# ZhonghuaYi/EI-Nexus_official

Hardware: AMD Instinct MI355X
Metric: event-image pairs/s (extract+match, 346x260, 1024 kpts) (higher is better)
Workload: dtype f32; 1 GPU; B32 346x260 5-bin event voxel + gray image, VGG(event)+SuperPoint(image) extractors, MNN matcher, k=1024; global_batch=32, event_bins=5, parallelism=dp1 (pairs sharded, metric all-reduce only), log_assignment=False, dense_outputs=False, same_scene_pairs=False, weights=seeded synthetic, descriptor-head bias calibrated (per-channel mean removed)

## Files before the change

### ei-nexus_official_amd/_lib.py

```python
import ctypes
import os

_HERE = os.path.dirname(os.path.abspath(__file__))
LIB_PATH = os.environ.get("EINX_LIB") or os.path.join(_HERE, "libeinx_hip.so")

c_void_p, c_int, c_float, c_size_t, c_char_p = ctypes.c_void_p, ctypes.c_int, ctypes.c_float, ctypes.c_size_t, ctypes.c_char_p


class ConvDesc(ctypes.Structure):
    _fields_ = [("w_native", c_void_p), ("bias", c_void_p), ("scale", c_void_p), ("shift", c_void_p),
                ("cin", ctypes.c_int32), ("cout", ctypes.c_int32), ("ks", ctypes.c_int32), ("relu", ctypes.c_int32),
                ("pool", ctypes.c_int32)]


class DetectParams(ctypes.Structure):
    _fields_ = [("B", ctypes.c_int32), ("Hp", ctypes.c_int32), ("Wp", ctypes.c_int32), ("H", ctypes.c_int32),
                ("W", ctypes.c_int32), ("h0", ctypes.c_int32), ("w0", ctypes.c_int32), ("radius", ctypes.c_int32),
                ("top_k", ctypes.c_int32), ("det_thr", c_float), ("ordering_xy", ctypes.c_int32), ("cap", ctypes.c_int32),
                ("nms_iters", ctypes.c_int32)]


class ExtractorDesc(ctypes.Structure):
    _fields_ = [("struct_size", c_size_t), ("cell", ctypes.c_int32), ("n_backbone", ctypes.c_int32), ("n_det", ctypes.c_int32), ("n_desc", ctypes.c_int32),
                ("backbone", ctypes.POINTER(ConvDesc)), ("det_head", ctypes.POINTER(ConvDesc)), ("desc_head", ctypes.POINTER(ConvDesc)),
# ... 34 lines not shown
class GtMatchesParams(ctypes.Structure):
    _fields_ = [("struct_size", c_size_t)] + [(n, ctypes.c_int32) for n in ("B", "cap0", "cap1", "cols0", "cols1", "kp_yx", "H0", "W0", "H1", "W1",
                                                                            "homography")] + [("pos_sq", c_float), ("neg_sq", c_float)]


class EventArrays(ctypes.Structure):
    _fields_ = [("x", c_void_p), ("y", c_void_p), ("t", c_void_p), ("p", c_void_p), ("x_type", ctypes.c_int32), ("y_type", ctypes.c_int32),
                ("t_type", ctypes.c_int32), ("p_type", ctypes.c_int32), ("n", ctypes.c_int64)]


class LgLayer(ctypes.Structure):
    _names = ("Wqkv", "bqkv", "Wo", "bo", "sf0_w", "sf0_b", "sln_g", "sln_b", "sf3_w", "sf3_b",
              "Wqk", "bqk", "Wv", "bv", "Wco", "bco", "cf0_w", "cf0_b", "cln_g", "cln_b", "cf3_w", "cf3_b", "Wqk_v", "bqk_v")
    _fields_ = [(n, c_void_p) for n in _names]


class LgWeights(ctypes.Structure):
    _fields_ = [("struct_size", c_size_t), ("layer_size", c_size_t), ("in_w", c_void_p), ("in_b", c_void_p), ("Wr", c_void_p), ("proj_w", c_void_p), ("proj_b", c_void_p),
                ("match_w", c_void_p), ("match_b", c_void_p), ("n_layers", ctypes.c_int32), ("heads", ctypes.c_int32),
                ("d", ctypes.c_int32), ("input_dim", ctypes.c_int32), ("filter_threshold", c_float),
                ("layers", ctypes.POINTER(LgLayer))]


class LgHead(ctypes.Structure):
    _fields_ = [(n, c_void_p) for n in ("proj_w", "proj_b", "match_w", "match_b", "token_w", "token_b")]


SIGNATURES = {
    "einx_version": (c_char_p, []),
    "einx_abi_version": (c_int, []),
    "einx_build_flags": (c_char_p, []),
    "einx_params_hash": (c_int, [c_void_p, c_int, c_void_p, c_void_p, c_void_p, c_void_p]),
    "einx_last_error": (c_char_p, []),
    "einx_math_eval": (c_int, [c_int, c_void_p, ctypes.c_longlong, c_void_p, c_void_p]),
    "einx_fork_stream_of": (c_void_p, [c_void_p]),
    "einx_fork_stream_prepare_beside": (c_int, [c_void_p, ctypes.POINTER(c_void_p), c_int]),
    "einx_stream_overlap_us": (c_int, [c_void_p, c_void_p, c_int, ctypes.POINTER(ctypes.c_float)]),
    "einx_device_count": (c_int, []),
    "einx_profile_enable": (c_int, [c_int]),
    "einx_profile_report": (c_int, [c_char_p, c_size_t]),
    "einx_extractor_create": (c_void_p, [ctypes.POINTER(ExtractorDesc)]),
    "einx_extractor_destroy": (None, [c_void_p]),
    "einx_fork_stream_prepare": (c_int, [c_void_p]),
    "einx_fork_stream_release": (c_int, [c_void_p]),
    "einx_fork_stream_count": (c_int, []),
    "einx_side_stream": (c_void_p, [c_void_p, c_int, ctypes.POINTER(c_void_p), c_int]),
    "einx_extract_shapes": (c_int, [c_void_p, c_int, c_int, ctypes.POINTER(ExtractShapes)]),
    "einx_extract_ws_bytes": (c_size_t, [c_void_p, c_int, c_int, c_int, c_int, c_int]),
    "einx_extract": (c_int, [c_void_p, c_void_p, c_void_p, c_int, c_int, c_int, c_int, c_void_p, c_size_t, ctypes.POINTER(ExtractOut), c_void_p]),
    "einx_extract_watch": (c_int, [c_void_p, c_void_p, c_void_p, c_int, c_int, c_int, c_int, c_void_p, c_size_t, ctypes.POINTER(ExtractOut),
                           ctypes.POINTER(WeightWatch), c_void_p]),
    "einx_conv_last_kernel": (c_char_p, []),
    "einx_conv_plan": (c_char_p, [c_int] * 11),
    "einx_conv_weight_elems": (c_size_t, [c_int, c_int, c_int]),
    "einx_conv_repack": (c_int, [c_void_p, c_int, c_int, c_int, c_void_p, c_void_p]),
    "einx_bn_fold": (c_int, [c_void_p, c_void_p, c_void_p, c_void_p, c_float, c_int, c_void_p, c_void_p, c_void_p]),
    "einx_conv_block": (c_int, [c_void_p, c_int, c_int, c_int, c_int, c_int, c_int, c_int, ctypes.POINTER(ConvDesc), c_void_p, c_void_p]),
    "einx_conv_first_two_fused_ok": (c_int, [ctypes.POINTER(ConvDesc), ctypes.POINTER(ConvDesc), c_int, c_int, c_int]),
    "einx_conv_first_two_fused": (c_int, [c_void_p, c_int, c_int, c_int, c_int, c_int, c_int, c_int, ctypes.POINTER(ConvDesc), ctypes.POINTER(ConvDesc),
                                  c_void_p, c_void_p]),
    "einx_div_inplace": (c_int, [c_void_p, c_size_t, c_float, c_void_p]),
    "einx_image_prepare": (c_int, [c_void_p, c_int, c_int, c_int, c_int, ctypes.c_longlong, ctypes.c_longlong, ctypes.c_longlong, ctypes.c_longlong,
                           c_float, c_void_p, c_void_p]),
    "einx_score_map": (c_int, [c_void_p, c_int, c_int, c_int, c_int, c_void_p, c_int, c_int, c_int, c_int, c_int, c_int, c_void_p,
                               c_void_p, c_void_p]),
    "einx_remove_border": (c_int, [c_void_p, c_int, c_int, c_int, c_int, c_void_p]),
    "einx_detect_ws_bytes": (c_size_t, [ctypes.POINTER(DetectParams)]),
    "einx_detect": (c_int, [c_void_p, ctypes.POINTER(DetectParams), c_void_p, c_void_p, c_void_p, c_void_p, c_void_p, c_void_p,
                            c_void_p, c_void_p]),
    "einx_desc_sample": (c_int, [c_void_p, c_int, c_int, c_int, c_int, c_int, c_int, c_int, c_int, c_void_p, c_void_p, c_int, c_float,
                                 c_void_p, c_void_p]),
    "einx_normalize_map": (c_int, [c_void_p, c_int, c_int, c_int, c_float, c_void_p, c_void_p, c_void_p]),
    "einx_upsample_ws_bytes": (c_size_t, [c_int, c_int, c_int]),
    "einx_upsample_normalize": (c_int, [c_void_p, c_int, c_int, c_int, c_int, c_int, c_int, c_int, c_int, c_int, c_int, c_float,
                                        c_void_p, c_void_p, c_size_t, c_void_p]),
    "einx_mnn_ws_bytes": (c_size_t, [c_int, c_int, c_int]),
    "einx_mnn": (c_int, [c_void_p, c_void_p, c_int, c_void_p, c_void_p, c_int, c_int, c_int, c_void_p, c_void_p, c_void_p, c_void_p,
                         c_void_p, c_void_p, c_void_p]),
    "einx_mnn_gather": (c_int, [c_void_p, c_void_p, c_int, c_void_p, c_void_p, c_int, c_int, c_int, c_void_p, c_void_p, c_void_p, c_void_p,
                                c_void_p, c_void_p, c_void_p, c_void_p, c_int, c_void_p, c_void_p, c_void_p, c_void_p]),
    "einx_mnn_thresh": (c_int, [c_void_p, c_void_p, c_int, c_void_p, c_void_p, c_int, c_int, c_int, c_int, c_float, c_int, c_float, c_void_p,
                                c_void_p, c_void_p, c_void_p, c_void_p, c_void_p, c_void_p]),
    "einx_gather_matches": (c_int, [c_void_p, c_void_p, c_void_p, c_void_p, c_int, c_int, c_int, c_int, c_void_p, c_void_p, c_void_p,
                                    c_void_p]),
    "einx_events_ws_bytes": (c_size_t, [c_int, c_int, c_int]),
    "einx_voxel_ws_bytes": (c_size_t, [c_int, c_int, c_int, c_int, ctypes.c_int64]),
    "einx_voxel_grid": (c_int, [c_void_p, c_void_p, c_void_p, c_void_p, c_void_p, c_int, c_int, c_int, c_int, c_int, c_void_p, c_void_p,
                                c_size_t, c_void_p]),
    "einx_events_mask": (c_int, [c_void_p, c_void_p, c_void_p, c_int, c_int, c_int, c_void_p, c_void_p, c_void_p]),
    "einx_time_surface_ws_bytes": (c_size_t, [c_int, c_int, c_int, c_int, ctypes.c_int64]),
    "einx_event_stack_ws_bytes": (c_size_t, [c_int, c_int, c_int, c_int, ctypes.c_int64]),
    "einx_distance_map_ws_bytes": (c_size_t, [c_int, c_int, c_int, c_int, ctypes.c_int64]),
    "einx_time_surface": (c_int, [c_void_p, c_void_p, c_void_p, c_void_p, c_void_p, c_int, c_int, c_int, c_int, c_void_p, c_void_p, c_size_t,
                                  c_void_p]),
    "einx_event_stack": (c_int, [c_void_p, c_void_p, c_void_p, c_void_p, c_void_p, c_int, c_int, c_int, c_int, c_void_p, c_void_p, c_size_t,
                                 c_void_p]),
    "einx_distance_map": (c_int, [c_void_p, c_void_p, c_void_p, c_void_p, c_void_p, c_int, c_int, c_int, c_int, c_void_p, c_void_p, c_size_t,
                                  c_void_p]),
    "einx_distance_map_plan": (c_char_p, [c_int, c_int]),
    "einx_events_windows_ws_bytes": (c_size_t, [c_int, c_int, c_int]),
    "einx_voxel_windows_ws_bytes": (c_size_t, [c_int, c_int, c_int, c_int, ctypes.c_int64]),
    "einx_voxel_grid_windows": (c_int, [c_void_p, c_void_p, c_void_p, c_void_p, ctypes.c_int64, c_void_p, c_void_p, c_int, c_int, c_int, c_int, c_int,
                                        c_void_p, c_void_p, c_size_t, c_void_p]),
    "einx_events_mask_windows": (c_int, [c_void_p, c_void_p, ctypes.c_int64, c_void_p, c_void_p, c_int, c_int, c_int, c_void_p, c_size_t, c_void_p,
                                         c_void_p]),
    "einx_events_pack": (c_int, [ctypes.POINTER(EventArrays), c_int, c_void_p, c_void_p, c_void_p, c_void_p, c_void_p, c_int]),
# ... 74 lines not shown
```

### ei-nexus_official_amd/csrc/conv.hip

```cpp
#include <stdio.h>
#include <stdlib.h>

#include <type_traits>

#include "einx_common.h"

namespace {

constexpr int kCoutTile = 64;

struct ConvArgs {
  const float* in;
  const float* w;
  const float* bias;
  const float* scale;
  const float* shift;
  float* out;
  int B, Cin, Cout, CoutPad;
  int Hs, Ws, h0, w0;
  int H, W;
  int tilesX, tilesY;
  int relu;
};

constexpr bool pitch_conflict_free(int th, int tw, int pitch) {
  const int npix = th * tw;
  for (int q0 = 0; q0 < npix; q0 += 32) {
    unsigned used = 0;
    for (int q = q0; q < q0 + 32 && q < npix; ++q) {
      const unsigned bit = 1u << (((q / tw) * pitch + q % tw) & 31);
      if (used & bit) return false;
      used |= bit;
    }
  }
  return true;
}
constexpr int conv_lds_pitch(int th, int tw) {
  for (int p = tw + 2; p < tw + 2 + 32; ++p)
    if (pitch_conflict_free(th, tw, p)) return p;
  return tw + 2;
}

template <int X>
__device__ __forceinline__ float lane_xor(float v) {
  const int i = __builtin_bit_cast(int, v);
  if constexpr (X == 1) return __builtin_bit_cast(float, __builtin_amdgcn_update_dpp(0, i, 0xB1, 0xF, 0xF, true));
  else if constexpr (X == 8) return __builtin_bit_cast(float, __builtin_amdgcn_update_dpp(0, i, 0x128, 0xF, 0xF, true));
  else if constexpr (X == 16) return __builtin_bit_cast(float, __builtin_amdgcn_ds_swizzle(i, 0x401F));
  else return __shfl_xor(v, X, 64);
}

template <int X>
__device__ __forceinline__ float max_lane_xor(float v) {
  if constexpr (X == 1) {
    float r;
    asm("s_nop 1\n\tv_max_f32_dpp %0, %1, %1 quad_perm:[1,0,3,2] row_mask:0xf bank_mask:0xf bound_ctrl:1" : "=v"(r) : "v"(v));
    return r;
  } else if constexpr (X == 8) {
    float r;
    asm("s_nop 1\n\tv_max_f32_dpp %0, %1, %1 row_ror:8 row_mask:0xf bank_mask:0xf bound_ctrl:1" : "=v"(r) : "v"(v));
    return r;
  } else {
    return fmaxf(v, lane_xor<X>(v));
  }
}

__device__ __forceinline__ __amdgpu_buffer_rsrc_t conv_rsrc(const void* p, unsigned bytes) {
  return __builtin_amdgcn_make_buffer_rsrc(const_cast<void*>(p), 0, (int)bytes, 0x00020000);
}

constexpr int conv_stage_groups(int nthr, int plane_e, int ck) {
  int ng = nthr / plane_e;
  while (ng > 1 && ck % ng != 0) --ng;
  return ng < 1 ? 1 : ng;
}

template <int KS, int TH, int TW, int WM, int WN, int MT, int NT, int CK, bool POOL, bool XTRA = false, int WPS = (CK < 8 ? 6 : 1)>
__global__ __launch_bounds__(WM * WN * 64, WPS) void conv_block_kernel(const ConvArgs a) {
  constexpr int kMT = MT, kNT = NT;
  constexpr int NW = WM * WN;
  constexpr int TAPS = KS * KS;
  constexpr int HALO = KS / 2;
  constexpr int PW = TW + 2 * HALO;
  constexpr int PH = TH + 2 * HALO;
  constexpr int PITCH = KS == 1 ? PW : conv_lds_pitch(TH, TW);
  constexpr int PLANE = PH * PITCH;
  constexpr int PLANE_E = PH * PW;
  constexpr int NTHR = NW * 64;
  constexpr int NPIX = TH * TW;
  static_assert(WM * MT * 32 == kCoutTile, "a workgroup covers 64 output channels");
  static_assert(WN * NT * 32 >= NPIX, "tile does not fit the workgroup's pixel slots");
  static_assert(KS == 1 || NPIX >= 32, "unused slots alias the slot one run earlier");
  static_assert(CK % 2 == 0, "channels are consumed in pairs");
  static_assert(PLANE_E <= NTHR, "one staging thread per halo position");
  constexpr int NG = conv_stage_groups(NTHR, PLANE_E, CK);
  constexpr int CPT = CK / NG;
  constexpr int IN_LDS = CK * PLANE;
  static_assert(IN_LDS % 4 == 0, "the weight tile behind the input tile is float4 aligned");
  constexpr int W_ROWS = CK * TAPS;
  constexpr int W_F4 = W_ROWS * kCoutTile / 4;
  constexpr int W_PER_THR = (W_F4 + NTHR - 1) / NTHR;
  constexpr int LDS_FLOATS = IN_LDS + W_ROWS * kCoutTile;

  __shared__ __attribute__((aligned(16))) float lds[LDS_FLOATS];
  __shared__ __attribute__((aligned(16))) float s_bias[kCoutTile], s_scale[kCoutTile], s_shift[kCoutTile];
  float* in_tile = lds;
  float* w_tile = lds + IN_LDS;

  const int tid = threadIdx.x;
  const int wave = __builtin_amdgcn_readfirstlane(tid >> 6);
  const int wm = wave / WN, wn = wave % WN;
  const int lane = tid & 63;
  const int half = lane >> 5;
  const int j = lane & 31;

  const int ncot = (int)gridDim.y;
  int item = xcd_contiguous((int)(blockIdx.x + blockIdx.y * gridDim.x), (int)gridDim.x * ncot);
  const int co0 = (item % ncot) * kCoutTile;
  int bid = item / ncot;
  const int tx_i = bid % a.tilesX;
  bid /= a.tilesX;
  const int ty_i = bid % a.tilesY;
  const int b = bid / a.tilesY;

  if (tid < kCoutTile) {
    const int co = co0 + tid;
    const bool cv = co < a.Cout;
    s_bias[tid] = (cv && a.bias) ? a.bias[co] : 0.0f;
    s_scale[tid] = (cv && a.scale) ? a.scale[co] : 1.0f;
    s_shift[tid] = (cv && a.scale) ? a.shift[co] : 0.0f;
// ... 59 lines not shown
  if (s_active && src_off < 0) {
#pragma unroll
    for (int i = 0; i < CPT; ++i) in_tile[lds_pos + i * PLANE] = 0.0f;
  }
  unsigned woff[W_PER_THR];
#pragma unroll
  for (int i = 0; i < W_PER_THR; ++i) {
    const int f = tid + i * NTHR;
    const int r = f / (kCoutTile / 4), c4 = f % (kCoutTile / 4);
    woff[i] = (unsigned)((f < W_F4 ? r : 0) * a.CoutPad + co0 + c4 * 4) * 4u;
  }

  f32x16 acc[kMT][kNT];
#pragma unroll
  for (int mt = 0; mt < kMT; ++mt)
#pragma unroll
    for (int nt = 0; nt < kNT; ++nt)
#pragma unroll
      for (int r = 0; r < 16; ++r) acc[mt][nt][r] = 0.0f;

  const int pairs_total = (a.Cin + 1) / 2;
  const int nchunks = (pairs_total * 2 + CK - 1) / CK;
  static_assert(!XTRA || (KS == 1 && NPIX <= NTHR && !POOL), "the extra channel is a 1x1 feature: one pixel per thread");
  float xacc = 0.0f;
  const bool xtra_wg = XTRA && co0 + kCoutTile == a.CoutPad - kCoutTile;

  struct StageRegs {
    float in[CPT];
    f32x4 w[W_PER_THR];
  };
  StageRegs sA;
  auto issue_loads = [&](int c) {
    const int ci0 = c * CK;
    if (s_ok) {
      const __amdgpu_buffer_rsrc_t rs = conv_rsrc(in_b + (size_t)ci0 * src_plane, (unsigned)(a.Cin - ci0) * src_plane * 4u);
#pragma unroll
      for (int i = 0; i < CPT; ++i) sA.in[i] = __builtin_bit_cast(float, __builtin_amdgcn_raw_buffer_load_b32(rs, in_voff[i], 0, 0));
    }
    const __amdgpu_buffer_rsrc_t rw = conv_rsrc(a.w + (size_t)c * W_ROWS * a.CoutPad, (unsigned)(W_ROWS * a.CoutPad) * 4u);
#pragma unroll
    for (int i = 0; i < W_PER_THR; ++i)
      if ((i + 1) * NTHR <= W_F4 || tid + i * NTHR < W_F4)
        sA.w[i] = __builtin_bit_cast(f32x4, __builtin_amdgcn_raw_buffer_load_b128(rw, woff[i], 0, 0));
  };
  auto commit_loads = [&]() {
    if (s_ok) {
#pragma unroll
      for (int i = 0; i < CPT; ++i) in_tile[lds_pos + i * PLANE] = sA.in[i];
    }
#pragma unroll
    for (int i = 0; i < W_PER_THR; ++i)
      if ((i + 1) * NTHR <= W_F4 || tid + i * NTHR < W_F4) *reinterpret_cast<f32x4*>(w_tile + (tid + i * NTHR) * 4) = sA.w[i];
  };
  auto mfma_chunk = [&]() {
    constexpr int STEPS = (CK / 2) * TAPS;
    constexpr int PF = 2;
    float av[PF + 1][kMT], bv[PF + 1][kNT];
    auto load_frag = [&](int st, int buf) {
      const int kp = st / TAPS, tap = st % TAPS;
      const int ky = tap / KS, kx = tap % KS;
#pragma unroll
      for (int mt = 0; mt < kMT; ++mt) av[buf][mt] = w_tile[aBase + (kp * TAPS + tap) * 2 * kCoutTile + mt * 32];
#pragma unroll
      for (int nt = 0; nt < kNT; ++nt) bv[buf][nt] = in_tile[bBase[nt] + kp * 2 * PLANE + ky * PITCH + kx];
    };
#pragma unroll
    for (int st = 0; st < PF && st < STEPS; ++st) load_frag(st, st % (PF + 1));
#pragma unroll
    for (int st = 0; st < STEPS; ++st) {
      if (st + PF < STEPS) load_frag(st + PF, (st + PF) % (PF + 1));
      __builtin_amdgcn_sched_barrier(0);
#pragma unroll
      for (int mt = 0; mt < kMT; ++mt)
#pragma unroll
        for (int nt = 0; nt < kNT; ++nt)
          acc[mt][nt] = __builtin_amdgcn_mfma_f32_32x32x2f32(av[st % (PF + 1)][mt], bv[st % (PF + 1)][nt], acc[mt][nt], 0, 0, 0);
      __builtin_amdgcn_sched_barrier(0);
    }
  };
  issue_loads(0);
  for (int c = 0; c < nchunks; ++c) {
    __syncthreads();
    commit_loads();
    __syncthreads();
    if (c + 1 < nchunks) issue_loads(c + 1);
    mfma_chunk();
    if (XTRA && xtra_wg && tid < NPIX) {
      const float* wx = a.w + (size_t)c * W_ROWS * a.CoutPad + (a.CoutPad - kCoutTile);
#pragma unroll
      for (int r = 0; r < CK; ++r) xacc = fmaf(wx[(size_t)r * a.CoutPad], in_tile[r * PLANE + tid], xacc);
    }
  }

  const int Ho = POOL ? a.H / 2 : a.H, Wo = POOL ? a.W / 2 : a.W;
  const unsigned plane_o = (unsigned)(Ho * Wo);
  float* out_b = a.out + (size_t)b * a.Cout * plane_o;
  if (XTRA && xtra_wg && tid < NPIX && p0 + tid < HW) {
    const int co = a.CoutPad - kCoutTile;
    float v = xacc + (a.bias ? a.bias[co] : 0.0f);
    if (a.relu) v = v > 0.0f ? v : 0.0f;
    if (a.scale) v = fmaf(v, a.scale[co], a.shift[co]);
    out_b[(size_t)co * HW + p0 + tid] = v;
  }
  static_assert(!POOL || TW == 32 || TW == 16 || TW == 8, "in-register pooling needs TW in {8,16,32}");
  static_assert(!POOL || TW != 32 || (NT % 2 == 0), "TW == 32 pools across N-tile pairs");
  constexpr int NO = (POOL && TW == 32) ? kNT / 2 : kNT;
  unsigned ovoff[NO];
#pragma unroll
  for (int o = 0; o < NO; ++o) {
    int pix;
    if (POOL) {
      pix = -1;
      const int q = qidx[(TW == 32) ? 2 * o : o];
      if (q >= 0) {
        const int ty = q / TW, tx = q % TW;
        const int yo = (y0 + ty) >> 1, xo = (x0 + tx) >> 1;
        if (!(ty & 1) && !(tx & 1) && yo < Ho && xo < Wo) pix = yo * Wo + xo;
// ... 587 lines not shown
      if (a.scale) v = fmaf(v, e_sc[i], e_sh[i]);
      if (co < a.Cout && p < HW) out_b[(size_t)co * HW + p] = v;
    }
  }
}

__global__ void conv_repack_kernel(const float* w, int cin, int cout, int taps, int coutPad, int krows, float* out) {
  const size_t n = (size_t)krows * coutPad;
  for (size_t i = (size_t)blockIdx.x * blockDim.x + threadIdx.x; i < n; i += (size_t)gridDim.x * blockDim.x) {
    const int co = (int)(i % coutPad);
    const int k = (int)(i / coutPad);
    const int h = k & 1;
    const int tap = (k >> 1) % taps;
    const int cp = (k >> 1) / taps;
    const int ci = 2 * cp + h;
    float v = 0.0f;
    if (ci < cin && co < cout) v = w[((size_t)co * cin + ci) * taps + tap];
    out[i] = v;
  }
}

__global__ void bn_fold_kernel(const float* g, const float* b, const float* mean, const float* var, float eps, int n, float* scale,
                               float* shift) {
  const int i = blockIdx.x * blockDim.x + threadIdx.x;
  if (i >= n) return;
  const float s = g[i] / sqrtf(var[i] + eps);
  scale[i] = s;
  shift[i] = b[i] - mean[i] * s;
}

int native_krows(int cin, int taps) { return einx_cdiv(cin, 32) * 32 * taps; }

thread_local const char* g_last_conv_kernel = "";

struct TileCfg {
  int th, tw, slots;
};

template <int KS, int TH, int TW, int WM, int WN, int MT, int NT, int CK, bool POOL, bool DENSE3 = false>
void launch(const ConvArgs& a, int B, hipStream_t s, bool three_per_cu = false) {
  dim3 grid((unsigned)(a.tilesX * a.tilesY * B), (unsigned)(a.CoutPad / kCoutTile));
  const bool three = DENSE3 && three_per_cu;
  {
    static char nm[2][96] = {{0}, {0}};
    char* n = nm[three ? 1 : 0];
    if (!n[0]) snprintf(n, sizeof nm[0], "conv_block_kernel<%d,%d,%d,%d,%d,%d,%d,%d,%s>%s", KS, TH, TW, WM, WN, MT, NT, CK, POOL ? "true" : "false", three ? " (3 per CU)" : "");
    g_last_conv_kernel = n;
  }
  EINX_PROF(KS == 1 ? "conv_block_kernel 1x1" : (CK < 8 ? "conv_block_kernel 3x3 first layer" : "conv_block_kernel 3x3"), s);
  if constexpr (DENSE3) {
    if (three) {
      hipLaunchKernelGGL((conv_block_kernel<KS, TH, TW, WM, WN, MT, NT, CK, POOL, false, 6>), grid, dim3(WM * WN * 64), 0, s, a);
      return;
    }
  }
  hipLaunchKernelGGL((conv_block_kernel<KS, TH, TW, WM, WN, MT, NT, CK, POOL>), grid, dim3(WM * WN * 64), 0, s, a);
}

double tile_waste(int H, int W, const TileCfg& c) {
  const double tiles = (double)einx_cdiv(H, c.th) * einx_cdiv(W, c.tw);
  return tiles * c.slots / ((double)H * W);
}

}

EINX_EXPORT const char* einx_conv_last_kernel(void) { return g_last_conv_kernel; }

EINX_EXPORT size_t einx_conv_weight_elems(int cin, int cout, int ks) {
  const int taps = ks * ks;
  const int coutPad = einx_cdiv(cout, kCoutTile) * kCoutTile;
  return (size_t)native_krows(cin, taps) * coutPad;
}

EINX_EXPORT int einx_conv_repack(const float* w_oihw, int cin, int cout, int ks, float* w_native, void* stream) {
  EINX_CHECK_ARG(w_oihw && w_native, "null pointer");
  EINX_CHECK_ARG(ks == 1 || ks == 3, "kernel size must be 1 or 3");
  EINX_CHECK_ARG(cin > 0 && cout > 0, "bad channel count");
  const int taps = ks * ks;
  const int coutPad = einx_cdiv(cout, kCoutTile) * kCoutTile;
  const int krows = native_krows(cin, taps);
  const size_t n = (size_t)krows * coutPad;
  const int blocks = (int)((n + 255) / 256 > 1024 ? 1024 : (n + 255) / 256);
  hipLaunchKernelGGL(conv_repack_kernel, dim3(blocks), dim3(256), 0, (hipStream_t)stream, w_oihw, cin, cout, taps, coutPad, krows,
                     w_native);
  EINX_CHECK_LAUNCH();
  return EINX_OK;
}

EINX_EXPORT int einx_bn_fold(const float* gamma, const float* beta, const float* mean, const float* var, float eps, int n, float* scale,
                             float* shift, void* stream) {
  EINX_CHECK_ARG(gamma && beta && mean && var && scale && shift, "null pointer");
  EINX_CHECK_ARG(n > 0, "bad channel count");
  hipLaunchKernelGGL(bn_fold_kernel, dim3(einx_cdiv(n, 256)), dim3(256), 0, (hipStream_t)stream, gamma, beta, mean, var, eps, n, scale,
                     shift);
  EINX_CHECK_LAUNCH();
  return EINX_OK;
}

EINX_EXPORT int einx_conv_first_two_fused_ok(const einx_conv_desc* d0, const einx_conv_desc* d1, int B, int H, int W) {
  if (!d0 || !d1) return 0;
  const bool shapes = (d0->cin == 1 || d0->cin == 5) && d0->cout == 64 && d0->ks == 3 && !d0->pool && d1->cin == 64 && d1->cout == 64 && d1->ks == 3;
  if (!shapes || (d1->pool && ((H & 1) || (W & 1)))) return 0;
  const long grid = (long)einx_cdiv(W, 32) * einx_cdiv(H, 8) * B;
  if (grid < 8L * 768) return 0;
  return d0->cin == 1 ? 1 : 2;
}
// ... 276 lines not shown
  a.H = H;
  a.W = W;
  a.relu = d->relu;
  const ConvPlan p = conv_plan(&pl, B, Hs, Ws, h0, w0, H, W);
  a.tilesX = p.tilesX;
  a.tilesY = p.tilesY;
  static thread_local char nm[96];
  switch (p.variant) {
#define X(V, KS, TH, TW, WM, WN, MT, NT, CK, POOL, DENSE3) \
  case V: launch<KS, TH, TW, WM, WN, MT, NT, CK, POOL, DENSE3>(a, B, s, p.three); break;
    EINX_CONV_BLOCK_VARIANTS(X)
#undef X
    case CB_1X1_128_XTRA: {
      dim3 grid((unsigned)(a.tilesX * B), (unsigned)(a.CoutPad / kCoutTile - 1));
      conv_plan_name(p, d->pool, nm, sizeof nm);
      g_last_conv_kernel = nm;
      EINX_PROF("conv_block_kernel 1x1", s);
      hipLaunchKernelGGL((conv_block_kernel<1, 1, 128, 1, 4, 2, 1, 32, false, true>), grid, dim3(256), 0, s, a);
      break;
    }
    case C16_1X1: {
      dim3 grid((unsigned)(a.tilesX * B), (unsigned)(a.CoutPad / kCoutTile));
      conv_plan_name(p, d->pool, nm, sizeof nm);
      g_last_conv_kernel = nm;
      EINX_PROF("conv16_1x1_kernel (small grid)", s);
      if (p.npw == 4) hipLaunchKernelGGL(conv16_1x1_kernel<4>, grid, dim3(256), 0, s, a);
      else if (p.npw == 2) hipLaunchKernelGGL(conv16_1x1_kernel<2>, grid, dim3(256), 0, s, a);
      else hipLaunchKernelGGL(conv16_1x1_kernel<1>, grid, dim3(256), 0, s, a);
      break;
    }
    default: {
      dim3 grid((unsigned)(a.tilesX * a.tilesY * B), (unsigned)(a.CoutPad / kCoutTile));
      conv_plan_name(p, d->pool, nm, sizeof nm);
      g_last_conv_kernel = nm;
      EINX_PROF("conv16_kernel 3x3 (small grid)", s);
#define EINX_C16(P, N) hipLaunchKernelGGL((conv16_kernel<P, 8, N>), grid, dim3(256), 0, s, a)
      if (d->pool) {
        if (p.npw == 4) EINX_C16(true, 4);
        else if (p.npw == 2) EINX_C16(true, 2);
        else EINX_C16(true, 1);
      } else {
        if (p.npw == 4) EINX_C16(false, 4);
        else if (p.npw == 2) EINX_C16(false, 2);
        else EINX_C16(false, 1);
      }
#undef EINX_C16
      break;
    }
  }
  EINX_CHECK_LAUNCH();
  return EINX_OK;
}

EINX_EXPORT const char* einx_conv_plan(int cin, int cout, int ks, int pool, int B, int Hs, int Ws, int h0, int w0, int H, int W) {
  const ConvPlanLayer pl = {cin, cout, ks, pool};
  if (const char* refused = conv_shape_refused(&pl, B, Hs, Ws, h0, w0, H, W)) {
    einx_set_error("%s: %s", __func__, refused);
    return nullptr;
  }
  static thread_local char nm[96];
  conv_plan_name(conv_plan(&pl, B, Hs, Ws, h0, w0, H, W), pool, nm, sizeof nm);
  return nm;
}
```

### ei-nexus_official_amd/csrc/detect.hip

```cpp
#include <algorithm>

#include "einx_common.h"

namespace {

__device__ __forceinline__ bool mask_on(const uint8_t* mask, int b, int H, int W, int h0, int w0, int Hp, int Wp, int y, int x,
                                        int dilate) {
  const int r = dilate ? 1 : 0;
  bool any = false;
#pragma unroll
  for (int dy = -1; dy <= 1; ++dy)
#pragma unroll
    for (int dx = -1; dx <= 1; ++dx) {
      const int yy = y + dy, xx = x + dx, sy = yy - h0, sx = xx - w0;
      const bool ok = dy >= -r && dy <= r && dx >= -r && dx <= r && yy >= 0 && yy < Hp && xx >= 0 && xx < Wp && sy >= 0 && sy < H && sx >= 0 && sx < W;
      const uint8_t m = mask[((size_t)b * H + min(max(sy, 0), H - 1)) * W + min(max(sx, 0), W - 1)];
      any |= ok && m != 0;
    }
  return any;
}

__global__ __launch_bounds__(256) void score65_kernel(const float* logits, int B, int hc, int wc, const uint8_t* mask, int H, int W,
                                                      int h0, int w0, int dilate, int border, float* prob, float* score, int32_t* zero_ptr,
                                                      int zero_n, float* crop) {
  if ((int)(blockIdx.x * 256 + threadIdx.x) < zero_n) zero_ptr[blockIdx.x * 256 + threadIdx.x] = 0;
  const int cells = hc * wc;
  const int lane = threadIdx.x & 63, wave = threadIdx.x >> 6;
  const int j = lane & 7, i = lane >> 3;
  const int gid = (blockIdx.x * 4 + wave) * 8 + j;
  const bool valid = gid < B * cells;
  const int g = valid ? gid : B * cells - 1;
  const int b = g / cells, cell = g % cells;
  const int h = cell / wc, w = cell % wc;
  const float* l = logits + (size_t)b * 65 * cells + cell;
  float v[8];
#pragma unroll
  for (int k = 0; k < 8; ++k) v[k] = l[(size_t)(8 * i + k) * cells];
  const float v64 = l[(size_t)64 * cells];
  float mx = v64;
#pragma unroll
  for (int k = 0; k < 8; ++k) mx = fmaxf(mx, v[k]);
  mx = fmaxf(mx, __shfl_xor(mx, 8, 64));
  mx = fmaxf(mx, __shfl_xor(mx, 16, 64));
  mx = fmaxf(mx, __shfl_xor(mx, 32, 64));
  float e[8];
#pragma unroll
  for (int k = 0; k < 8; ++k) e[k] = einx_expf(v[k] - mx);
  const float e64 = einx_expf(v64 - mx);
  float s = 0.0f;
#pragma unroll
  for (int c = 0; c < 64; ++c) s = s + __shfl(e[c & 7], j + 8 * (c >> 3), 64);
  s = s + e64;
  if (!valid) return;
  const int Hp = hc * 8, Wp = wc * 8;
  float* pr = prob + (size_t)b * 65 * cells + cell;
  const int y = h * 8 + i;
  unsigned cols = 0x3ffu;
  if (mask) {
    cols = 0;
    const int r = dilate ? 1 : 0;
#pragma unroll
    for (int dy = -1; dy <= 1; ++dy) {
      const int yy = y + dy, sy = yy - h0;
      const bool rok = dy >= -r && dy <= r && yy >= 0 && yy < Hp && sy >= 0 && sy < H;
      const uint8_t* mrow = mask + ((size_t)b * H + min(max(sy, 0), H - 1)) * W;
      uint8_t m[10];
#pragma unroll
      for (int k = 0; k < 10; ++k) m[k] = mrow[min(max(w * 8 - 1 + k - w0, 0), W - 1)];
#pragma unroll
      for (int k = 0; k < 10; ++k) {
        const int xx = w * 8 - 1 + k, sx = xx - w0;
        if (rok && xx >= 0 && xx < Wp && sx >= 0 && sx < W && m[k]) cols |= 1u << k;
      }
    }
  }
  const unsigned window = (mask && !dilate) ? 2u : 7u;
  float out[8];
#pragma unroll
  for (int k = 0; k < 8; ++k) {
    const float p = e[k] / s;
    pr[(size_t)(8 * i + k) * cells] = p;
    const int x = w * 8 + k;
    float t = p;
    if (!((cols >> k) & window)) t = 0.0f;
    if (border > 0 && (y < border || y >= Hp - border || x < border || x >= Wp - border)) t = 0.0f;
    out[k] = t;
  }
  if (i == 0) pr[(size_t)64 * cells] = e64 / s;
  f32x4* dst = reinterpret_cast<f32x4*>(score + ((size_t)b * Hp + y) * Wp + w * 8);
  dst[0] = f32x4{out[0], out[1], out[2], out[3]};
  dst[1] = f32x4{out[4], out[5], out[6], out[7]};
  if (crop) {
    const int uy = y - h0;
    if (uy >= 0 && uy < H) {
      float* cr = crop + ((size_t)b * H + uy) * W - w0 + w * 8;
#pragma unroll
      for (int k = 0; k < 8; ++k) {
        const int ux = w * 8 + k - w0;
        if (ux >= 0 && ux < W) cr[k] = out[k];
      }
    }
  }
}

__global__ void score1_kernel(const float* logits, int B, int Hp, int Wp, const uint8_t* mask, int H, int W, int h0, int w0,
                              int dilate, int border, float* prob, float* score, int32_t* zero_ptr, int zero_n, float* crop) {
  const int n = Hp * Wp;
  const int gid = blockIdx.x * blockDim.x + threadIdx.x;
  if (gid < zero_n) zero_ptr[gid] = 0;
  if (gid >= B * n) return;
  const int b = gid / n, p = gid % n;
  const int y = p / Wp, x = p % Wp;
  float v = einx_sigmoidf(logits[gid]);
  if (mask && !mask_on(mask, b, H, W, h0, w0, Hp, Wp, y, x, dilate)) v = 0.0f;
  if (border > 0 && (y < border || y >= Hp - border || x < border || x >= Wp - border)) v = 0.0f;
  prob[gid] = v;
  score[gid] = v;
  if (crop) {
    const int uy = y - h0, ux = x - w0;
    if (uy >= 0 && uy < H && ux >= 0 && ux < W) crop[((size_t)b * H + uy) * W + ux] = v;
  }
}

__global__ void dense_positions_kernel(const float* score, int B, int H, int W, int xy, float* out) {
  const size_t n = (size_t)B * H * W;
  const size_t gid = (size_t)blockIdx.x * blockDim.x + threadIdx.x;
  if (gid >= n) return;
  const int p = (int)(gid % ((size_t)H * W));
  const float fy = (float)(p / W) + 0.5f, fx = (float)(p % W) + 0.5f;
// ... 705 lines not shown
      keep = v > thr && uy >= 0 && uy < a.H && ux >= 0 && ux < a.W;
    }
    int total;
    const int pos = base + block_excl_scan(keep ? 1 : 0, &total, scratch);
    if (keep && pos < a.cap) {
      const float py = ((float)y + 0.5f) - (float)a.h0, px = ((float)x + 0.5f) - (float)a.w0;
      float* o = a.positions + ((size_t)b * a.cap + pos) * 3;
      o[0] = a.ordering_xy ? px : py;
      o[1] = a.ordering_xy ? py : px;
      o[2] = v;
      a.indices[(size_t)b * a.cap + pos] = fi;
    }
    base += total;
  }
  if (tid == 0) a.counts[b] = base;
}

__global__ void nms_crop_kernel(const float* map, const float* thr, int B, int Hp, int Wp, int h0, int w0, int H, int W, float* out) {
  const size_t n = (size_t)B * H * W;
  const size_t gid = (size_t)blockIdx.x * blockDim.x + threadIdx.x;
  if (gid >= n) return;
  const int b = (int)(gid / ((size_t)H * W));
  const int r = (int)(gid % ((size_t)H * W));
  const float v = map[((size_t)b * Hp + (r / W + h0)) * Wp + r % W + w0];
  out[gid] = v > thr[b] ? v : 0.0f;
}

void topk_ranks(int N, int k, int* lo, int* hi) {
  const float q = (float)(N - k) / (float)N;
  const float rank = q * (float)(N - 1);
  *lo = (int)floorf(rank);
  *hi = (int)ceilf(rank);
}

}

EINX_EXPORT int einx_score_map(const float* logits, int B, int C, int hc, int wc, const uint8_t* mask, int H, int W, int h0, int w0,
                               int dilate, int border, float* prob, float* score, void* stream) {
  return einx_score_map_zero(logits, B, C, hc, wc, mask, H, W, h0, w0, dilate, border, prob, score, nullptr, 0, nullptr, stream);
}

int einx_score_map_zero(const float* logits, int B, int C, int hc, int wc, const uint8_t* mask, int H, int W, int h0, int w0, int dilate,
                        int border, float* prob, float* score, int32_t* zero_ptr, int zero_n, float* crop, void* stream) {
  EINX_CHECK_ARG(!crop || (H > 0 && W > 0), "the cropped map needs the un-padded size");
  EINX_CHECK_ARG(logits && prob && score, "null pointer");
  EINX_CHECK_ARG(zero_n == 0 || (zero_ptr && (long)zero_n <= (long)(C == 65 ? einx_cdiv(B * hc * wc, 32) : einx_cdiv(B * hc * wc, 256)) * 256),
                 "more words to zero than threads in the launch");
  EINX_CHECK_ARG(C == 65 || C == 1, "detector head must have 65 or 1 channels");
  EINX_CHECK_ARG(B > 0 && hc > 0 && wc > 0, "bad shape");
  hipStream_t s = (hipStream_t)stream;
  EINX_PROF("score_map (score65/score1)", s);
  if (C == 65) {
    const int n = B * hc * wc;
    hipLaunchKernelGGL(score65_kernel, dim3(einx_cdiv(n, 32)), dim3(256), 0, s, logits, B, hc, wc, mask, H, W, h0, w0, dilate, border,
                       prob, score, zero_ptr, zero_n, crop);
  } else {
    const int n = B * hc * wc;
    hipLaunchKernelGGL(score1_kernel, dim3(einx_cdiv(n, 256)), dim3(256), 0, s, logits, B, hc, wc, mask, H, W, h0, w0, dilate, border,
                       prob, score, zero_ptr, zero_n, crop);
  }
  EINX_CHECK_LAUNCH();
  return EINX_OK;
}

EINX_EXPORT int einx_remove_border(float* score, int B, int Hp, int Wp, int border, void* stream) {
  EINX_CHECK_ARG(score, "null pointer");
  if (border <= 0) return EINX_OK;
  const int n = B * Hp * Wp;
  hipLaunchKernelGGL(border_kernel, dim3(einx_cdiv(n, 256)), dim3(256), 0, (hipStream_t)stream, score, B, Hp, Wp, border);
  EINX_CHECK_LAUNCH();
  return EINX_OK;
}

EINX_EXPORT int einx_dense_positions(const float* score, int B, int H, int W, int ordering_xy, float* out, void* stream) {
  EINX_CHECK_ARG(score && out, "null pointer");
  EINX_CHECK_ARG(B > 0 && H > 0 && W > 0, "bad shape");
  const size_t n = (size_t)B * H * W;
  hipLaunchKernelGGL(dense_positions_kernel, dim3((unsigned)((n + 255) / 256)), dim3(256), 0, (hipStream_t)stream, score, B, H, W, ordering_xy, out);
  EINX_CHECK_LAUNCH();
  return EINX_OK;
}

EinxDetectWs einx_detect_carve(WsCarver& c, const einx_detect_params* p) {
  const size_t map = (size_t)p->B * p->Hp * p->Wp;
  const EinxDetectWs w{c.take<float>(map), c.take<float>(map), c.take<int32_t>((size_t)p->B * (p->nms_iters > 0 ? p->nms_iters : 1)),
                       p->radius > 0 ? p->B * p->nms_iters : 0};
  c.slack(256);
  return w;
}

EINX_EXPORT size_t einx_detect_ws_bytes(const einx_detect_params* p) {
  if (!p) return 0;
  WsCarver c{nullptr};
  einx_detect_carve(c, p);
  return c.bytes;
}

EINX_EXPORT int einx_detect(const float* score, const einx_detect_params* p, void* ws, float* nms_out, float* positions,
                            int32_t* indices, int32_t* counts, float* thr, int32_t* not_converged, void* stream) {
  return einx_detect_prezeroed(score, p, ws, nms_out, positions, indices, counts, thr, not_converged, 0, nullptr, stream);
}

int einx_detect_prezeroed(const float* score, const einx_detect_params* p, void* ws, float* nms_out, float* positions, int32_t* indices,
                          int32_t* counts, float* thr, int32_t* not_converged, int flags_zeroed, const float** final_map, void* stream) {
  EINX_CHECK_ARG(score && p && ws && positions && indices && counts && thr && not_converged, "null pointer");
  EINX_CHECK_ARG(p->B > 0 && p->Hp > 0 && p->Wp > 0 && p->cap > 0, "bad shape");
  EINX_CHECK_ARG(p->radius >= 0 && p->radius <= NMS_MAXR, "nms radius must be in 0..4");
  EINX_CHECK_ARG(p->radius == 0 || p->nms_iters >= 1, "nms_iters must be >= 1");
// ... 73 lines not shown
```

### include/einx.h

```cpp
#ifndef EINX_H
#define EINX_H

#include <stddef.h>
#include <stdint.h>

#ifdef __cplusplus
extern "C" {
#endif

#define EINX_OK 0
#define EINX_ERR_ARG (-1)
#define EINX_ERR_LAUNCH (-2)
#define EINX_ERR_NO_DEVICE (-3)

#define EINX_ABI_VERSION 6
int einx_abi_version(void);
const char* einx_version(void);
const char* einx_last_error(void);
const char* einx_build_flags(void);
int einx_device_count(void);

#define EINX_WATCH_CHUNK_WORDS 4096
int einx_params_hash(const int64_t* table, int n, uint64_t* hash, const uint64_t* ref, int32_t* stale, void* stream);

int einx_math_eval(int fn, const float* x, long long n, float* y, void* stream);

int einx_stream_overlap_us(void* stream_a, void* stream_b, int spin_us, float* elapsed_us);

int einx_profile_enable(int on);
int einx_profile_report(char* buf, size_t cap);


size_t einx_conv_weight_elems(int cin, int cout, int ks);
int einx_conv_repack(const float* w_oihw, int cin, int cout, int ks, float* w_native, void* stream);

int einx_bn_fold(const float* gamma, const float* beta, const float* mean, const float* var, float eps, int n, float* scale,
                 float* shift, void* stream);

typedef struct einx_conv_desc {
  const float* w_native;
  const float* bias;
  const float* scale;
  const float* shift;
  int32_t cin, cout, ks;
  int32_t relu;
  int32_t pool;
} einx_conv_desc;

int einx_conv_block(const float* in, int B, int Hs, int Ws, int h0, int w0, int H, int W, const einx_conv_desc* d, float* out,
                    void* stream);

int einx_conv_first_two_fused_ok(const einx_conv_desc* d0, const einx_conv_desc* d1, int B, int H, int W);
int einx_conv_first_two_fused(const float* in, int B, int Hs, int Ws, int h0, int w0, int H, int W, const einx_conv_desc* d0,
                              const einx_conv_desc* d1, float* out, void* stream);

const char* einx_conv_last_kernel(void);

const char* einx_conv_plan(int cin, int cout, int ks, int pool, int B, int Hs, int Ws, int h0, int w0, int H, int W);

int einx_div_inplace(float* x, size_t n, float divisor, void* stream);

int einx_image_prepare(float* image, int B, int C, int H, int W, long long stride_b, long long stride_c, long long stride_h,
                       long long stride_w, float divisor, float* gray, void* stream);


int einx_score_map(const float* logits, int B, int C, int hc, int wc, const uint8_t* mask, int H, int W, int h0, int w0,
                   int dilate, int border, float* prob, float* score, void* stream);

int einx_remove_border(float* score, int B, int Hp, int Wp, int border, void* stream);

int einx_dense_positions(const float* score, int B, int H, int W, int ordering_xy, float* out, void* stream);

typedef struct einx_detect_params {
  int32_t B, Hp, Wp;
  int32_t H, W, h0, w0;
  int32_t radius;
  int32_t top_k;
  float det_thr;
  int32_t ordering_xy;
  int32_t cap;
  int32_t nms_iters;
} einx_detect_params;

size_t einx_detect_ws_bytes(const einx_detect_params* p);

int einx_detect(const float* score, const einx_detect_params* p, void* ws, float* nms_out, float* positions, int32_t* indices,
                int32_t* counts, float* thr, int32_t* not_converged, void* stream);


int einx_desc_sample(const float* raw, int B, int D, int hc, int wc, int Hp, int Wp, int bilinear, int channels_last,
                     const int32_t* indices, const int32_t* counts, int cap, float scale, float* out, void* stream);

int einx_normalize_map(const float* raw, int B, int D, int P, float scale, float* out, float* raw_cl, void* stream);

int einx_normalize_rows(const float* x, int R, int C, float scale, float* out, void* stream);

int einx_random_positions(const float* u, int R, float size0, float size1, float* out, void* stream);

size_t einx_upsample_ws_bytes(int B, int H, int W);
int einx_upsample_normalize(const float* raw, int B, int D, int hc, int wc, int Hp, int Wp, int h0, int w0, int H, int W,
                            float scale, float* out, void* ws, size_t ws_bytes, void* stream);

size_t einx_mnn_ws_bytes(int B, int cap0, int cap1);
int einx_mnn(const float* desc0, const int32_t* n, int cap0, const float* desc1, const int32_t* m, int cap1, int B, int D,
             void* ws, int64_t* matches0, int64_t* matches1, float* scores0, float* scores1, float* la, void* stream);
int einx_mnn_gather(const float* desc0, const int32_t* n, int cap0, const float* desc1, const int32_t* m, int cap1, int B, int D,
                    void* ws, int64_t* matches0, int64_t* matches1, float* scores0, float* scores1, float* la, const float* kpts0,
                    const float* kpts1, int cols, float* mk0, float* mk1, int32_t* nmatch, void* stream);
int einx_mnn_thresh(const float* desc0, const int32_t* n, int cap0, const float* desc1, const int32_t* m, int cap1, int B, int D,
                    int use_ratio, float ratio_sq, int use_dist, float dist_sq, void* ws, int64_t* matches0, int64_t* matches1,
                    float* scores0, float* scores1, float* la, void* stream);
// ... 258 lines not shown
```

Baseline: 3823 pairs/s.

## Pack odd-channel tail taps in thin convs and ballot-precompute score mask bits

For the thin first conv layers, where Cin is odd and smaller than the chunk, the MFMA walk now folds the last unpaired channel's taps two at a time into one pair step. This cuts the zero-padded MFMA steps over the dummy channel. Separately, score65 is templated on whether a mask is present. With a mask, each block first builds a shared-memory bitmask of the 10 mask rows using wave ballots, so threads no longer do per-thread byte gathers. Both changes add index complexity and more template instantiations, and the mask path adds a __syncthreads and extra shared memory.

```diff
diff --git a/ei-nexus_official_amd/_lib.py b/ei-nexus_official_amd/_lib.py
--- a/ei-nexus_official_amd/_lib.py
+++ b/ei-nexus_official_amd/_lib.py
@@ -110,6 +110,7 @@
                            ctypes.POINTER(WeightWatch), c_void_p]),
     "einx_conv_last_kernel": (c_char_p, []),
     "einx_conv_plan": (c_char_p, [c_int] * 11),
+    "einx_conv_thin_steps": (c_int, [c_int, c_int, c_int, ctypes.POINTER(c_int), c_int]),
     "einx_conv_weight_elems": (c_size_t, [c_int, c_int, c_int]),
     "einx_conv_repack": (c_int, [c_void_p, c_int, c_int, c_int, c_void_p, c_void_p]),
     "einx_bn_fold": (c_int, [c_void_p, c_void_p, c_void_p, c_void_p, c_float, c_int, c_void_p, c_void_p, c_void_p]),
diff --git a/ei-nexus_official_amd/csrc/conv.hip b/ei-nexus_official_amd/csrc/conv.hip
--- a/ei-nexus_official_amd/csrc/conv.hip
+++ b/ei-nexus_official_amd/csrc/conv.hip
@@ -75,7 +75,18 @@
   return ng < 1 ? 1 : ng;
 }
 
-template <int KS, int TH, int TW, int WM, int WN, int MT, int NT, int CK, bool POOL, bool XTRA = false, int WPS = (CK < 8 ? 6 : 1)>
+struct ThinStep {
+  int pair, tap0, tap1;
+};
+constexpr int thin_steps(int ck, int taps, int np) { return np < 0 ? (ck / 2) * taps : np * taps + (taps + 1) / 2; }
+constexpr int thin_np(int ck, int cin) { return ((cin & 1) && cin < ck) ? cin >> 1 : -1; }
+constexpr ThinStep thin_step(int taps, int np, int st) {
+  if (np < 0 || st < np * taps) return {st / taps, st % taps, -1};
+  const int t = 2 * (st - np * taps);
+  return {np, t, t + 1 < taps ? t + 1 : -1};
+}
+
+template <int KS, int TH, int TW, int WM, int WN, int MT, int NT, int CK, bool POOL, bool XTRA = false, int WPS = (CK < 8 ? 6 : 1), int NP = -1>
 __global__ __launch_bounds__(WM * WN * 64, WPS) void conv_block_kernel(const ConvArgs a) {
   constexpr int kMT = MT, kNT = NT;
   constexpr int NW = WM * WN;
@@ -241,17 +252,35 @@
     for (int i = 0; i < W_PER_THR; ++i)
       if ((i + 1) * NTHR <= W_F4 || tid + i * NTHR < W_F4) *reinterpret_cast<f32x4*>(w_tile + (tid + i * NTHR) * 4) = sA.w[i];
   };
+  static_assert(NP < 0 || (KS == 3 && CK < 8 && 2 * NP + 1 < CK), "the packed walk is the thin first layers'");
+  const int aPack = aBase + half * kCoutTile;
+  int bPackCol[kNT], bPackRow[kNT];
+#pragma unroll
+  for (int nt = 0; nt < kNT; ++nt) {
+    bPackCol[nt] = bBase[nt] - half * PLANE + half;
+    bPackRow[nt] = bBase[nt] - half * PLANE + half * (PITCH - (KS - 1));
+  }
   auto mfma_chunk = [&]() {
-    constexpr int STEPS = (CK / 2) * TAPS;
+    constexpr int STEPS = thin_steps(CK, TAPS, NP);
     constexpr int PF = 2;
     float av[PF + 1][kMT], bv[PF + 1][kNT];
     auto load_frag = [&](int st, int buf) {
-      const int kp = st / TAPS, tap = st % TAPS;
-      const int ky = tap / KS, kx = tap % KS;
-#pragma unroll
-      for (int mt = 0; mt < kMT; ++mt) av[buf][mt] = w_tile[aBase + (kp * TAPS + tap) * 2 * kCoutTile + mt * 32];
-#pragma unroll
-      for (int nt = 0; nt < kNT; ++nt) bv[buf][nt] = in_tile[bBase[nt] + kp * 2 * PLANE + ky * PITCH + kx];
+      const ThinStep ts = thin_step(TAPS, NP, st);
+      if (ts.tap1 < 0) {
+        const int kp = ts.pair, tap = ts.tap0;
+        const int ky = tap / KS, kx = tap % KS;
+#pragma unroll
+        for (int mt = 0; mt < kMT; ++mt) av[buf][mt] = w_tile[aBase + (kp * TAPS + tap) * 2 * kCoutTile + mt * 32];
+#pragma unroll
+        for (int nt = 0; nt < kNT; ++nt) bv[buf][nt] = in_tile[bBase[nt] + kp * 2 * PLANE + ky * PITCH + kx];
+      } else {
+        const int tap = ts.tap0, ky = tap / KS, kx = tap % KS;
+#pragma unroll
+        for (int mt = 0; mt < kMT; ++mt) av[buf][mt] = w_tile[aPack + (ts.pair * TAPS + tap) * 2 * kCoutTile + mt * 32];
+#pragma unroll
+        for (int nt = 0; nt < kNT; ++nt)
+          bv[buf][nt] = in_tile[(kx == KS - 1 ? bPackRow[nt] : bPackCol[nt]) + ts.pair * 2 * PLANE + ky * PITCH + kx];
+      }
     };
 #pragma unroll
     for (int st = 0; st < PF && st < STEPS; ++st) load_frag(st, st % (PF + 1));
@@ -945,6 +974,26 @@
     if (three) {
       hipLaunchKernelGGL((conv_block_kernel<KS, TH, TW, WM, WN, MT, NT, CK, POOL, false, 6>), grid, dim3(WM * WN * 64), 0, s, a);
       return;
+    }
+  }
+  if constexpr (KS == 3 && CK < 8) {
+    constexpr int WPS = 6;
+    const int np = thin_np(CK, a.Cin);
+    if (np == 0) {
+      hipLaunchKernelGGL((conv_block_kernel<KS, TH, TW, WM, WN, MT, NT, CK, POOL, false, WPS, 0>), grid, dim3(WM * WN * 64), 0, s, a);
+      return;
+    }
+    if constexpr (CK >= 4) {
+      if (np == 1) {
+        hipLaunchKernelGGL((conv_block_kernel<KS, TH, TW, WM, WN, MT, NT, CK, POOL, false, WPS, 1>), grid, dim3(WM * WN * 64), 0, s, a);
+        return;
+      }
+    }
+    if constexpr (CK >= 6) {
+      if (np == 2) {
+        hipLaunchKernelGGL((conv_block_kernel<KS, TH, TW, WM, WN, MT, NT, CK, POOL, false, WPS, 2>), grid, dim3(WM * WN * 64), 0, s, a);
+        return;
+      }
     }
   }
   hipLaunchKernelGGL((conv_block_kernel<KS, TH, TW, WM, WN, MT, NT, CK, POOL>), grid, dim3(WM * WN * 64), 0, s, a);
@@ -1327,6 +1376,16 @@
   return EINX_OK;
 }
 
+EINX_EXPORT int einx_conv_thin_steps(int cin, int ck, int taps, int* steps, int cap) {
+  EINX_CHECK_ARG(cin > 0 && ck > 0 && ck < 8 && ck % 2 == 0 && cin <= ck && taps > 0 && (steps || cap == 0), "bad argument");
+  const int np = thin_np(ck, cin), n = thin_steps(ck, taps, np);
+  for (int i = 0; i < n && i < cap; ++i) {
+    const ThinStep ts = thin_step(taps, np, i);
+    steps[3 * i] = ts.pair, steps[3 * i + 1] = ts.tap0, steps[3 * i + 2] = ts.tap1;
+  }
+  return n;
+}
+
 EINX_EXPORT const char* einx_conv_plan(int cin, int cout, int ks, int pool, int B, int Hs, int Ws, int h0, int w0, int H, int W) {
   const ConvPlanLayer pl = {cin, cout, ks, pool};
   if (const char* refused = conv_shape_refused(&pl, B, Hs, Ws, h0, w0, H, W)) {
diff --git a/ei-nexus_official_amd/csrc/detect.hip b/ei-nexus_official_amd/csrc/detect.hip
--- a/ei-nexus_official_amd/csrc/detect.hip
+++ b/ei-nexus_official_amd/csrc/detect.hip
@@ -20,6 +20,10 @@
   return any;
 }
 
+constexpr int kScoreCells = 32;
+__device__ __forceinline__ int score_seg_words(int n) { return (8 * n + 2 + 63) >> 6; }
+
+template <bool MASK>
 __global__ __launch_bounds__(256) void score65_kernel(const float* logits, int B, int hc, int wc, const uint8_t* mask, int H, int W,
                                                       int h0, int w0, int dilate, int border, float* prob, float* score, int32_t* zero_ptr,
                                                       int zero_n, float* crop) {
@@ -37,6 +41,53 @@
 #pragma unroll
   for (int k = 0; k < 8; ++k) v[k] = l[(size_t)(8 * i + k) * cells];
   const float v64 = l[(size_t)64 * cells];
+  __shared__ unsigned long long s_bits[10][kScoreCells + 1];
+  const int Hp = hc * 8, Wp = wc * 8;
+  const int g0 = blockIdx.x * kScoreCells;
+  const int R0 = g0 / wc, wfirst = g0 - R0 * wc;
+  int words0 = 0, words_full = 0;
+  if constexpr (MASK) {
+    const int glast = min(g0 + kScoreCells, B * cells) - 1;
+    const int R1 = glast / wc;
+    words0 = score_seg_words(min(wc - wfirst, glast - g0 + 1));
+    words_full = score_seg_words(wc);
+    const int words_all = R1 == R0 ? words0 : words0 + (R1 - R0 - 1) * words_full + score_seg_words(glast - R1 * wc + 1);
+    const int uwave = __builtin_amdgcn_readfirstlane(wave);
+    for (int wd0 = uwave; wd0 < words_all; wd0 += 8) {
+      uint8_t m[2][10];
+      bool cok[2];
+      int sy0[2];
+#pragma unroll
+      for (int u = 0; u < 2; ++u) {
+        const int wd = min(wd0 + 4 * u, words_all - 1);
+        const int sg = wd < words0 ? 0 : 1 + (wd - words0) / words_full;
+        const int k = wd < words0 ? wd : (wd - words0) - (sg - 1) * words_full;
+        const int R = R0 + sg;
+        const int sb = R / hc, sh = R - sb * hc;
+        const int wa = sg == 0 ? wfirst : 0, wb = R == R1 ? glast - R * wc : wc - 1;
+        const int t = k * 64 + lane;
+        const int xx = wa * 8 - 1 + t, sx = xx - w0;
+        cok[u] = (t < 8 * (wb - wa + 1) + 2) & (xx >= 0) & (xx < Wp) & (sx >= 0) & (sx < W);
+        sy0[u] = sh * 8 - 1 - h0;
+        const uint8_t* mcol = mask + (size_t)sb * H * W + min(max(sx, 0), W - 1);
+#pragma unroll
+        for (int r = 0; r < 10; ++r) m[u][r] = mcol[(size_t)min(max(sy0[u] + r, 0), H - 1) * W];
+      }
+#pragma unroll
+      for (int u = 0; u < 2; ++u) {
+        unsigned long long mine = 0;
+#pragma unroll
+        for (int r = 0; r < 10; ++r) {
+          const int sy = sy0[u] + r, yy = sy + h0;
+          const bool rok = (yy >= 0) & (yy < Hp) & (sy >= 0) & (sy < H);
+          const unsigned long long bal = __ballot((int)(cok[u] & rok & (m[u][r] != 0)));
+          mine = lane == r ? bal : mine;
+        }
+        if (wd0 + 4 * u < words_all && lane < 10) s_bits[lane][wd0 + 4 * u] = mine;
+      }
+    }
+    __syncthreads();
+  }
   float mx = v64;
 #pragma unroll
   for (int k = 0; k < 8; ++k) mx = fmaxf(mx, v[k]);
@@ -52,29 +103,23 @@
   for (int c = 0; c < 64; ++c) s = s + __shfl(e[c & 7], j + 8 * (c >> 3), 64);
   s = s + e64;
   if (!valid) return;
-  const int Hp = hc * 8, Wp = wc * 8;
   float* pr = prob + (size_t)b * 65 * cells + cell;
   const int y = h * 8 + i;
   unsigned cols = 0x3ffu;
-  if (mask) {
+  if constexpr (MASK) {
+    const int sg = b * hc + h - R0;
+    const int bit = 64 * (sg == 0 ? 0 : words0 + (sg - 1) * words_full) + 8 * (w - (sg == 0 ? wfirst : 0));
     cols = 0;
-    const int r = dilate ? 1 : 0;
 #pragma unroll
     for (int dy = -1; dy <= 1; ++dy) {
-      const int yy = y + dy, sy = yy - h0;
-      const bool rok = dy >= -r && dy <= r && yy >= 0 && yy < Hp && sy >= 0 && sy < H;
-      const uint8_t* mrow = mask + ((size_t)b * H + min(max(sy, 0), H - 1)) * W;
-      uint8_t m[10];
-#pragma unroll
-      for (int k = 0; k < 10; ++k) m[k] = mrow[min(max(w * 8 - 1 + k - w0, 0), W - 1)];
-#pragma unroll
-      for (int k = 0; k < 10; ++k) {
-        const int xx = w * 8 - 1 + k, sx = xx - w0;
-        if (rok && xx >= 0 && xx < Wp && sx >= 0 && sx < W && m[k]) cols |= 1u << k;
-      }
-    }
-  }
-  const unsigned window = (mask && !dilate) ? 2u : 7u;
+      if (dy != 0 && !dilate) continue;
+      const unsigned* row = reinterpret_cast<const unsigned*>(s_bits[i + 1 + dy]);
+      const unsigned long long two = ((unsigned long long)row[(bit >> 5) + 1] << 32) | row[bit >> 5];
+      cols |= (unsigned)(two >> (bit & 31));
+    }
+    cols &= 0x3ffu;
+  }
+  const unsigned window = (MASK && !dilate) ? 2u : 7u;
   float out[8];
 #pragma unroll
   for (int k = 0; k < 8; ++k) {
@@ -886,8 +931,13 @@
   EINX_PROF("score_map (score65/score1)", s);
   if (C == 65) {
     const int n = B * hc * wc;
-    hipLaunchKernelGGL(score65_kernel, dim3(einx_cdiv(n, 32)), dim3(256), 0, s, logits, B, hc, wc, mask, H, W, h0, w0, dilate, border,
-                       prob, score, zero_ptr, zero_n, crop);
+    EINX_CHECK_ARG(!mask || (H > 0 && W > 0), "the events mask needs the un-padded size");
+    if (mask)
+      hipLaunchKernelGGL(score65_kernel<true>, dim3(einx_cdiv(n, kScoreCells)), dim3(256), 0, s, logits, B, hc, wc, mask, H, W, h0, w0, dilate,
+                         border, prob, score, zero_ptr, zero_n, crop);
+    else
+      hipLaunchKernelGGL(score65_kernel<false>, dim3(einx_cdiv(n, kScoreCells)), dim3(256), 0, s, logits, B, hc, wc, mask, H, W, h0, w0, dilate,
+                         border, prob, score, zero_ptr, zero_n, crop);
   } else {
     const int n = B * hc * wc;
     hipLaunchKernelGGL(score1_kernel, dim3(einx_cdiv(n, 256)), dim3(256), 0, s, logits, B, hc, wc, mask, H, W, h0, w0, dilate, border,
diff --git a/include/einx.h b/include/einx.h
--- a/include/einx.h
+++ b/include/einx.h
@@ -57,6 +57,8 @@
 const char* einx_conv_last_kernel(void);
 
 const char* einx_conv_plan(int cin, int cout, int ks, int pool, int B, int Hs, int Ws, int h0, int w0, int H, int W);
+
+int einx_conv_thin_steps(int cin, int ck, int taps, int* steps, int cap);
 
 int einx_div_inplace(float* x, size_t n, float divisor, void* stream);
 
```

New measurement: 3822 pairs/s. Within noise of the previous version (-0.0%).
